# CUHK-SE-Group/MicroRank

Hardware: AMD Instinct MI355X
Metric: PageRank GTEPS + RCA windows ranked/sec at 1/2/4/8 MI355X; % HBM roofline (higher is better)
Workload: dtype f64

## Files before the change

microrank_amd/csrc/mr_graph_build.hip:

```cpp
#include <algorithm>
#include <cstring>
#include <vector>

#include "mr_detect_dev.h"
#include "mr_prim.h"
#include "mr_sort.h"

namespace {
constexpr int BT = 256;
constexpr int LDS_HIST = 8192;
constexpr int ESET = 1024;
constexpr uint64_t EMPTY = ~0ull;

__device__ __forceinline__ uint64_t hmix(uint64_t z) {
    z ^= z >> 33;
    z *= 0xff51afd7ed558ccdull;
    z ^= z >> 33;
    z *= 0xc4ceb9fe1a85ec53ull;
    return z ^ (z >> 33);
}

__global__ void k_count_codes(const int64_t* span, int64_t S, int32_t* cnt) {
    int64_t i = (int64_t)blockIdx.x * blockDim.x + threadIdx.x;
    if (i < S) atomicAdd(&cnt[span[i]], 1);
// ... 1920 lines not shown
    for (int k = 0; k < n; ++k) as.w[k].st = dst + woff[(size_t)k];
    if (fuse) {
        hipLaunchKernelGGL(k_ix_detect_scan2_b, dim3(bs), dim3(DB), 0, st, as, epoch);
    } else {
        if (dets) {
            int32_t bd = 0;
            IxBatch<IxWinSel> ad = as;
            for (int k = 0; k < n; ++k) {
                ad.b0[k] = bd;
                bd += (int32_t)cdiv((int64_t)sps[k]->n_traces, DB);
            }
            for (int k = n; k <= IXW; ++k) ad.b0[k] = bd;
            if (bd) hipLaunchKernelGGL(k_ix_detect_b, dim3(bd), dim3(DB), 0, st, ad);
        }
        hipLaunchKernelGGL(k_ix_sel_scan2_b, dim3(bs), dim3(SEL_T), 0, st, as, epoch);
    }
    if (bt) hipLaunchKernelGGL(k_ix_stats2_b, dim3(bt), dim3(IX_BT), lds, st, at);
    if (bc) hipLaunchKernelGGL(k_ix_cross2_b, dim3(bc), dim3(256), 0, st, ac);
    hipLaunchKernelGGL(k_nodes_small2_b, dim3(2 * n), dim3(NS_T), 0, st, an);
    if (br) hipLaunchKernelGGL(k_ix_traces2_b, dim3(br), dim3(256), 0, st, ar);
    MR_TRY_HIP(ctx, hipGetLastError());
    return MR_OK;
}

constexpr int LB_T = 512;
constexpr int64_t LB_LDS_WORDS = 30720;
constexpr int32_t LB_A3MAX = 4096;
bool mr_lo_fits(const mr_spans* sp) {
    return sp->indexed && sp->ekey.p && sp->n_podops <= NS_PMAX && sp->n_edge_keys <= NS_EMAX &&
           2 * (3 * (int64_t)sp->n_podops + sp->n_edge_keys) + 2 * (int64_t)sp->n_svcops <= LB_LDS_WORDS &&
           sp->n_svcops <= LB_A3MAX && sp->n_traces <= (1 << 24);
}
struct IxWinLoB {
    const int32_t *lo_tr, *lo_len, *lo_kid, *lo_first, *bstart;
    const int64_t *lo_off, *lsv_off, *le_off;
    const uint16_t *lo16, *lo_cnt;
    const uint32_t *lsv, *le;
    const long long *lo_ts, *lo_te, *lo_mx;
    const double* a3;
    const uint8_t* a3v;
    int64_t t0, t1;
    uint8_t* state;
    int8_t* side;
    unsigned long long* counts;
    int32_t NT, NP, nek, nsvc;
    uint32_t* kcnt[2];
    int64_t* tot[2];
    uint32_t* rows;
};
__host__ __device__ __forceinline__ size_t lo_region0(size_t gbytes) {
    return 2 * gbytes > (size_t)2048 * 8 ? 2 * gbytes : (size_t)2048 * 8;
}
constexpr int LB_R = 4;
__device__ __forceinline__ int32_t lo_trace_of(uint32_t e, uint32_t n, const uint32_t* st, int32_t nt) {
    if (n > 0) return (int32_t)(e / n);
    int32_t lo = 0;
#pragma unroll
    for (int32_t step = LO_BT_MAX / 2; step >= 1; step >>= 1) {
        const int32_t mid = lo + step;
        lo = mid < nt && st[mid] <= e ? mid : lo;
    }
    return lo;
}
__global__ void __launch_bounds__(LB_T, 6) k_lo_build_b(IxBatch<IxWinLoB> a) {
    extern __shared__ __attribute__((aligned(16))) unsigned char lraw[];
    __shared__ uint32_t pst[LO_BT_MAX + 1], est[LO_BT_MAX + 1];
    __shared__ int8_t ss[LO_BT_MAX];
    __shared__ unsigned long long bc[5][LB_T / WAVE];
    const int k = ixb_pick(a.b0, a.n);
    const IxWinLoB& w = a.w[k];
    const int32_t blk = (int32_t)blockIdx.x - a.b0[k];
    const int tid = threadIdx.x, lane = tid & (WAVE - 1), wv = tid / WAVE;
    const int32_t NP = w.NP, nek = w.nek;
    const size_t gbytes = ((size_t)NP * 12 + (size_t)nek * 4 + 15) / 16 * 16;
    const size_t reg0 = lo_region0(gbytes);
    double* la3 = (double*)(lraw + reg0);
    double* prod = (double*)lraw;
    const uint32_t cap = (uint32_t)(reg0 / 8 / LB_T * LB_T);
    for (int32_t c = tid; c < w.nsvc; c += LB_T) la3[c] = w.a3v[c] ? w.a3[c] : 0.0;
    const int32_t T0 = w.bstart[blk], nt = w.bstart[blk + 1] - T0;
    const int64_t P0 = w.lo_off[T0], Q0 = w.le_off[T0], V0 = w.lsv_off[T0];
    const uint32_t np = (uint32_t)(w.lo_off[T0 + nt] - P0), nq = (uint32_t)(w.le_off[T0 + nt] - Q0);
    const uint32_t nv = (uint32_t)(w.lsv_off[T0 + nt] - V0);
    if (tid == 0) {
        pst[nt] = np;
        est[nt] = nq;
    }
    constexpr int NS = LO_BT_MAX / LB_T;
    uint32_t va[NS], vb[NS];
    bool act[NS];
    double expect[NS];
    long long mx[NS];
    unsigned long long rows = 0;
#pragma unroll
    for (int q = 0; q < NS; ++q) {
        const int32_t t = q * LB_T + tid;
        const bool valid = t < nt;
        const int64_t i = (int64_t)T0 + (valid ? t : nt - 1);
        const int32_t len = w.lo_len[i];
        const long long ts = w.lo_ts[i], te = w.lo_te[i];
        mx[q] = w.lo_mx[i];
        va[q] = (uint32_t)(w.lsv_off[i] - V0);
        vb[q] = (uint32_t)(w.lsv_off[i + 1] - V0);
        const bool in = valid && len > 0 && ts >= w.t0 && te <= w.t1;
        rows += in ? (unsigned long long)len : 0ull;
        act[q] = in && mx[q] > 0;
        expect[q] = 0.0;
    }
    __syncthreads();
    for (uint32_t r0 = 0; r0 < nv; r0 += cap) {
        const uint32_t rn = min(cap, nv - r0);
        constexpr int LU = 8;
        for (uint32_t x0 = 0; x0 < rn; x0 += LU * LB_T) {
            uint32_t v[LU];
#pragma unroll
            for (int u = 0; u < LU; ++u) {
                const uint32_t x = x0 + (uint32_t)(u * LB_T + tid);
                v[u] = w.lsv[V0 + (int64_t)(r0 + min(x, rn - 1))];
            }
#pragma unroll
            for (int u = 0; u < LU; ++u) {
                const uint32_t x = x0 + (uint32_t)(u * LB_T + tid);
                if (x < rn) prod[x] = (double)(v[u] >> 16) * la3[v[u] & 0xffffu];
            }
        }
        __syncthreads();
#pragma unroll
        for (int q = 0; q < NS; ++q)
            if (act[q]) {
                const uint32_t lo = max(va[q], r0), hi = min(vb[q], r0 + rn);
                for (uint32_t j = lo; j < hi; j += 8) {
                    double p8[8];
#pragma unroll
                    for (int u = 0; u < 8; ++u) p8[u] = prod[min(j + u, hi - 1) - r0];
#pragma unroll
                    for (int u = 0; u < 8; ++u)
                        if (j + u < hi) expect[q] += p8[u];
                }
            }
        __syncthreads();
    }
    for (size_t x = (size_t)tid * 4; x < reg0; x += (size_t)LB_T * 4) *(uint32_t*)(lraw + x) = 0u;
    unsigned long long nab = 0, nno = 0, nz0 = 0, nz1 = 0;
#pragma unroll
    for (int q = 0; q < NS; ++q) {
        const int32_t t = q * LB_T + tid;
        const bool valid = t < nt;
        const int64_t i = (int64_t)T0 + (valid ? t : nt - 1);
        const int32_t kid0 = w.lo_kid[i], tr = w.lo_tr[i];
        const int64_t pa = w.lo_off[i], pb = w.lo_off[i + 1], ea = w.le_off[i];
        const int stt = act[q] ? ((double)mx[q] / 1000.0 > expect[q] ? 2 : 1) : 0;
        const int s_ = valid ? (stt == 2 ? 0 : stt == 1 ? 1 : -1) : -1;
        if (valid) {
            w.state[tr] = (uint8_t)stt;
            w.side[i] = (int8_t)s_;
            ss[t] = (int8_t)s_;
            pst[t] = (uint32_t)(pa - P0);
            est[t] = (uint32_t)(ea - Q0);
        }
        nab += stt == 2;
        nno += stt == 1;
        if (s_ == 0) nz0 += (unsigned long long)(pb - pa);
        else if (s_ == 1) nz1 += (unsigned long long)(pb - pa);
        const int kid = valid ? kid0 : -1;
        const int kp = __shfl_up(kid, 1, WAVE);
        const bool hd = kid >= 0 && (lane == 0 || kp != kid);
        const unsigned long long H = __ballot(hd), B0 = __ballot(s_ == 0), B1 = __ballot(s_ == 1);
        if (hd) {
            const unsigned long long above = lane == WAVE - 1 ? 0ull : H & (~0ull << (lane + 1));
            const unsigned long long run = (above ? (above & (0ull - above)) - 1ull : ~0ull) & (~0ull << lane);
            const uint32_t c0 = (uint32_t)__popcll(B0 & run), c1 = (uint32_t)__popcll(B1 & run);
            if (c0) atomicAdd(&w.kcnt[0][kid], c0);
            if (c1) atomicAdd(&w.kcnt[1][kid], c1);
        }
    }
    __syncthreads();
    constexpr int LB_LANE = 8;
    const bool lanewise = nt > 0 && pst[nt] - pst[nt - 1] <= (uint32_t)LB_LANE;
    if (lanewise) {
#pragma unroll
        for (int q = 0; q < NS; ++q) {
            const int32_t t = q * LB_T + tid;
            const int sd = t < nt ? (int)ss[t] : -1;
            if (sd < 0) continue;
            unsigned char* G = lraw + (size_t)sd * gbytes;
            const uint32_t a0 = pst[t], n = pst[t + 1] - a0, rot = n ? (uint32_t)t % n : 0u;
            uint32_t pc[LB_LANE];
            int32_t fr[LB_LANE];
#pragma unroll
            for (int u = 0; u < LB_LANE; ++u) {
                const uint32_t j = (uint32_t)u + rot;
                const int64_t e = P0 + (int64_t)a0 + (u < (int)n ? (j >= n ? j - n : j) : 0u);
                pc[u] = (uint32_t)w.lo16[e] | ((uint32_t)w.lo_cnt[e] << 16);
                fr[u] = w.lo_first[e];
            }
#pragma unroll
            for (int u = 0; u < LB_LANE; ++u)
                if (u < (int)n) {
                    const uint32_t c = pc[u] & 0xffffu;
                    atomicAdd((unsigned long long*)G + c, (unsigned long long)(pc[u] >> 16) | (1ull << 32));
                    atomicMax((int32_t*)(G + (size_t)NP * 8) + c, 0x7fffffff - fr[u]);
                }
            const uint32_t b0e = est[t], m = est[t + 1] - b0e, rte = m ? (uint32_t)t % m : 0u;
            uint32_t* Ge = (uint32_t*)(G + (size_t)NP * 12);
            for (uint32_t u0 = 0; u0 < m; u0 += LB_LANE) {
                uint32_t ev[LB_LANE];
#pragma unroll
                for (int u = 0; u < LB_LANE; ++u) {
                    const uint32_t j = u0 + (uint32_t)u, jr = j + rte;
                    ev[u] = w.le[Q0 + (int64_t)b0e + (j < m ? (jr >= m ? jr - m : jr) : 0u)];
                }
#pragma unroll
                for (int u = 0; u < LB_LANE; ++u)
                    if (u0 + (uint32_t)u < m) atomicAdd(Ge + (ev[u] & 0xffffu), ev[u] >> 16);
            }
        }
    }
    const uint32_t n0 = nt ? pst[1 < nt ? 1 : nt] - pst[0] : 0u;
    const uint32_t npo = n0 > 0 && np == (uint32_t)nt * n0 ? n0 : 0u;
    constexpr int NW = LB_T / WAVE;
    const uint32_t nmax = lanewise ? 0u : max(np, nq);
    for (uint32_t b0 = (uint32_t)wv * (LB_R * WAVE); b0 < nmax; b0 += NW * LB_R * WAVE) {
        uint32_t pc[LB_R], ev[LB_R];
        int32_t fr[LB_R];
#pragma unroll
        for (int r = 0; r < LB_R; ++r) {
            const uint32_t o = b0 + (uint32_t)(r * WAVE + lane);
            if (b0 < np) {
                const int64_t e = P0 + (int64_t)min(o, np - 1u);
                pc[r] = (uint32_t)w.lo16[e] | ((uint32_t)w.lo_cnt[e] << 16);
                fr[r] = w.lo_first[e];
            }
            if (b0 < nq) ev[r] = w.le[Q0 + (int64_t)min(o, nq - 1u)];
        }
#pragma unroll
        for (int r = 0; r < LB_R; ++r) {
            const uint32_t o = b0 + (uint32_t)(r * WAVE + lane);
            if (o < np) {
                const int sd = ss[lo_trace_of(o, npo, pst, nt)];
                if (sd >= 0) {
                    unsigned char* G = lraw + (size_t)sd * gbytes;
                    const uint32_t c = pc[r] & 0xffffu;
                    atomicAdd((unsigned long long*)G + c, (unsigned long long)(pc[r] >> 16) | (1ull << 32));
                    atomicMax((int32_t*)(G + (size_t)NP * 8) + c, 0x7fffffff - fr[r]);
                }
            }
            if (o < nq) {
                const int sd = ss[lo_trace_of(o, 0u, est, nt)];
                if (sd >= 0)
                    atomicAdd((uint32_t*)(lraw + (size_t)sd * gbytes + (size_t)NP * 12) + (ev[r] & 0xffffu), ev[r] >> 16);
            }
        }
    }
    __syncthreads();
    {
        unsigned long long v[5] = {nab, nno, rows, nz0, nz1};
#pragma unroll
        for (int m = 32; m >= 1; m >>= 1)
#pragma unroll
            for (int q = 0; q < 5; ++q) v[q] += __shfl_xor(v[q], m, WAVE);
        if (lane == 0)
#pragma unroll
            for (int q = 0; q < 5; ++q) bc[q][wv] = v[q];
    }
    __syncthreads();
    if (tid < 5) {
        unsigned long long v = 0;
        for (int q = 0; q < NW; ++q) v += bc[tid][q];
        if (v) {
            if (tid < 3) atomicAdd(&w.counts[(size_t)(blk % CSH) * 3 + tid], v);
            else atomicAdd((unsigned long long*)&w.tot[tid - 3][1], v);
        }
    }
    const size_t rw = 3 * (size_t)NP + (size_t)nek;
    uint32_t* R = w.rows + (size_t)blk * 2 * rw;
    for (int g = 0; g < 2; ++g) {
        const unsigned char* G = lraw + (size_t)g * gbytes;
        uint32_t* Rg = R + (size_t)g * rw;
// ... 170 lines not shown
            ap.w[k].tot[j] = out + 5;
            L.kcnt[j] = B.kcnt;
            L.tot[j] = out + 5;
            IxLoRed& R = ar.w[k];
            R.ocnt[j] = ocnt;
            R.ofinv[j] = ofinv;
            R.ocov[j] = ocov;
            R.gc[j] = gc;
        }
        const int32_t nt = sp->lo_nblk;
        const int64_t rw = 3 * (int64_t)NP + nek;
        roff[(size_t)k] = rwords;
        rwords += (int64_t)nt * 2 * rw;
        ar.w[k].nblk = nt;
        ar.w[k].NP = NP;
        ar.w[k].nek = (int32_t)nek;
        ar.b0[k] = br;
        br += (int32_t)cdiv(2 * rw, 256);
        const int32_t npb = (int32_t)std::max<int64_t>(cdiv((int64_t)NT, LP_TILE), 1);
        woff[(size_t)k] = words;
        words += 2 * (int64_t)npb;
        ap.b0[k] = bp;
        bp += npb;
        ap.w[k].NT = NT;
        soff[(size_t)k] = sbytes;
        sbytes += ((int64_t)NT + 15) / 16 * 16;
        ab.b0[k] = bb;
        bb += nt;
        const DetIn& d = dets[k];
        L.bstart = sp->lo_bstart.p;
        L.lo_tr = sp->lo_tr.p;
        L.lo_len = sp->lo_len.p;
        L.lo_kid = sp->lo_kid.p;
        L.lo_first = sp->lo_first.p;
        L.lo_off = sp->lo_off.p;
        L.lsv_off = sp->lsv_off.p;
        L.le_off = sp->le_off.p;
        L.lo16 = sp->lo16.p;
        L.lo_cnt = sp->lo_cnt.p;
        L.lsv = sp->lsv.p;
        L.le = sp->le.p;
        L.lo_ts = sp->lo_ts.p;
        L.lo_te = sp->lo_te.p;
        L.lo_mx = sp->lo_mx.p;
        L.a3 = d.a3;
        L.a3v = d.a3v;
        L.t0 = d.t0;
        L.t1 = d.t1;
        L.state = d.state;
        L.counts = d.counts;
        L.NT = NT;
        L.NP = NP;
        L.nek = (int32_t)nek;
        L.nsvc = sp->n_svcops;
        lds = std::max(lds, lo_region0(((size_t)NP * 12 + (size_t)nek * 4 + 15) / 16 * 16) + (size_t)sp->n_svcops * 8);
        ac.b0[k] = bc;
        bc += (int32_t)cdiv(sp->n_xj, 256);
        ac.w[k] = IxWinCross{d.state, sp->xj_tc.p, sp->xj_tp.p, sp->xj_eid.p, sp->n_xj, xs};
        an.b0[k] = 2 * k;
        an.w[k] = IxWinNodes{sp->ekey.p, nek, NP, 0, na};
    }
    for (int k = n; k <= IXW; ++k) {
        ab.b0[k] = bb;
        ar.b0[k] = br;
        ap.b0[k] = bp;
        ac.b0[k] = bc;
        an.b0[k] = 2 * n;
    }
    unsigned long long* dst = nullptr;
    uint64_t epoch = 0;
    MR_TRY(mr_dl_status(ctx, words, &dst, &epoch));
    DBuf<uint32_t> rows;
    DBuf<int8_t> side;
    MR_TRY(rows.alloc(ctx, (size_t)std::max<int64_t>(rwords, 1)));
    MR_TRY(side.alloc(ctx, (size_t)std::max<int64_t>(sbytes, 16)));
    for (int k = 0; k < n; ++k) {
        ab.w[k].rows = rows.p + roff[(size_t)k];
        ar.w[k].rows = rows.p + roff[(size_t)k];
        ab.w[k].side = side.p + soff[(size_t)k];
        ap.w[k].side = side.p + soff[(size_t)k];
        ap.w[k].st = dst + woff[(size_t)k];
    }
    hipLaunchKernelGGL(k_lo_build_b, dim3(bb), dim3(LB_T), lds, st, ab);
    hipLaunchKernelGGL(k_lo_pos_b, dim3(bp), dim3(LP_T), 0, st, ap, epoch);
    hipLaunchKernelGGL(k_lo_reduce_b, dim3(br), dim3(256), 0, st, ar);
    if (bc) hipLaunchKernelGGL(k_ix_cross2_b, dim3(bc), dim3(256), 0, st, ac);
    hipLaunchKernelGGL(k_nodes_small2_b, dim3(2 * n), dim3(NS_T), 0, st, an);
    MR_TRY_HIP(ctx, hipGetLastError());
// ... 112 lines not shown
```

microrank_amd/csrc/mr_internal.h:

```cpp
#pragma once
#include <hip/hip_runtime.h>

#include <cstdarg>
#include <cstdint>
#include <cstdio>
#include <map>
#include <string>
#include <unordered_map>
#include <utility>
#include <memory>
#include <mutex>
#include <vector>

#include "../../include/microrank_hip.h"

constexpr int WAVE = 64;

struct mr_ctx {
    int device = 0;
    hipStream_t stream = nullptr;
    uint32_t flags = 0;
    std::string err;
    void* comm = nullptr;
    int rank = 0, nranks = 1;
// ... 236 lines not shown
    mr_ctx* ctx = nullptr;
    int64_t S = 0;
    int32_t n_traces = 0, n_podops = 0, n_svcops = 0;
    DBuf<int32_t> trace, podop, svcop;
    DBuf<int64_t> span, parent, duration, tstart, tend;
    bool has_times = false;
    DBuf<int32_t> grow;
    int row_bits = 0;
    int64_t n_span_codes = 0;
    DBuf<int64_t> id_off;
    DBuf<int32_t> id_rows;
    bool indexed = false;
    bool uniform_times = false;
    DBuf<int32_t> tlen;
    DBuf<long long> tmaxd, tts, tte;
    int64_t n_po = 0, n_sv = 0, n_ed = 0, n_xj = 0;
    int64_t n_edge_keys = 0;
    DBuf<uint64_t> ekey;
    DBuf<int32_t> ed_eid, xj_eid;
    DBuf<int64_t> po_off;
    DBuf<int32_t> po_op, po_cnt, po_first, po_tr;
    DBuf<int64_t> sv_off;
    DBuf<int32_t> sv_op, sv_cnt;
    DBuf<int64_t> ed_off;
    DBuf<uint64_t> ed_key;
    DBuf<int32_t> ed_cnt, ed_tr;
    DBuf<int32_t> eb_tr, eb_cnt, eb_eid;
    DBuf<int32_t> xj_tc, xj_tp;
    DBuf<uint64_t> xj_key;
    bool lo_ok = false;
    int32_t lo_nk = 0;
    DBuf<int32_t> lo_tr, lo_len, lo_kid;
    DBuf<int64_t> lo_off;
    DBuf<uint16_t> lo16, lo_cnt;
    DBuf<int32_t> lo_first;
    DBuf<long long> lo_ts, lo_te, lo_mx;
    DBuf<int32_t> lo_bstart;
    int32_t lo_nblk = 0;
    DBuf<int64_t> lsv_off, le_off;
    DBuf<uint32_t> lsv, le;
    DBuf<int32_t> dict_rows[3];
    bool raw = false;
    DBuf<int64_t> raw_off[6];
    DBuf<uint8_t> raw_bytes[6], raw_valid;
    DBuf<int64_t> src;
    int64_t src_next = 0;
};

int mr_spans_index(mr_ctx* ctx, mr_spans* s);

void mr_handle_add(mr_ctx* ctx, void* h, void (*del)(void*));
bool mr_handle_take(void* h);

enum { MR_DT_F64 = 0, MR_DT_I32 = 1, MR_DT_U64 = 2, MR_DT_I64 = 3 };
int mr_coll_allreduce(mr_ctx* ctx, void* dbuf, int64_t n, int dtype, int op );
int mr_coll_allgather(mr_ctx* ctx, const void* dsend, void* drecv, int64_t n, int dtype);
inline bool mr_coll_ready(const mr_ctx* ctx) { return ctx->comm || ctx->host_coll; }
int mr_peer_allreduce_u64(mr_ctx* ctx, unsigned long long* dbuf, int64_t n);
int mr_peer_allreduce_f64(mr_ctx* ctx, double* dbuf, int64_t n);
int mr_peer_check(mr_ctx* ctx, const char* what);
struct MrPeerX {
    unsigned long long* const* peers;
    unsigned long long* region;
    int32_t R, rank, nbf, spin;
    int32_t mute;
    int64_t slots, W, bflags, err;
    uint64_t seq;
    unsigned long long timeout;
// ... 46 lines not shown
int mr_pagerank_batch_async(mr_ctx* ctx, mr_graph* const* gs, const int* anomaly, int ng, double d, double alpha,
                            int iters, int precision, int32_t* hflag, PrAsync** out, bool defer = false);
int mr_pagerank_async_commit(mr_ctx* ctx, PrAsync* a);
int mr_pagerank_async_finish(mr_ctx* ctx, PrAsync* a, bool* rerun);
void mr_pagerank_async_free(PrAsync* a);
int mr_ix_launch2_batch(mr_ctx* ctx, int n, const mr_spans* const* sps, uint8_t* const* d_states, mr_graph* const* g0s,
                        mr_graph* const* g1s, IxBuild* const* b0s, IxBuild* const* b1s, int64_t* const* d_outs,
                        const DetIn* dets, bool fuse);
constexpr int MR_DETECT_SHARDS = 64;
int mr_detect_indexed_launch(mr_ctx* ctx, const mr_spans* s, int64_t t0, int64_t t1, const double* d_a3,
                             const uint8_t* d_a3v, uint8_t* d_state, unsigned long long* counts);
void mr_detect_sum(const unsigned long long* sh, int32_t* n_abn, int32_t* n_nor, int64_t* n_in);
int mr_detect_sweep_launch(mr_ctx* ctx, const mr_spans* s, int64_t t_begin, int64_t grain, int64_t window, int32_t M,
                           const double* d_a3, const uint8_t* d_a3v, uint8_t* d_state, unsigned long long* diff);
constexpr size_t MR_WS_SLOT = 12 * 256 + 16;
int mr_win_spectrum_launch(mr_ctx* ctx, int32_t Na, const int32_t* a_podop, const double* a_w, const int32_t* a_cov,
                           int32_t Nn, const int32_t* n_podop, const double* n_w, const int32_t* n_cov, int32_t NP,
                           int64_t A, int64_t Nl, int method, int32_t k, unsigned char* d_slot);
void mr_win_spectrum_unpack(const unsigned char* slot, int32_t* out_codes, double* out_score, int32_t* n_out);
constexpr int MR_WS_BATCH = 8;
struct MrWsWin {
    const int32_t *a_podop, *a_cov, *n_podop, *n_cov;
    const double *a_w, *n_w;
    unsigned char* out;
    int64_t A, Nl;
    int32_t Na, Nn, NP;
};
bool mr_win_spectrum_fits(int32_t Na, int32_t Nn, int32_t NP, int32_t k);
int mr_win_spectrum_launch_n(mr_ctx* ctx, const MrWsWin* ws, int n, int method, int32_t k);
int mr_ix_finish(mr_ctx* ctx, const mr_spans* sp, mr_graph* g, IxBuild& b, const int64_t* h);
bool mr_lo_fits(const mr_spans* sp);
constexpr int32_t LO_BT_MAX = 1024;
constexpr int64_t LO_BE = 12288;
int64_t mr_lo_zero_words(const mr_spans* sp);
int mr_lo_launch_batch(mr_ctx* ctx, int n, const mr_spans* const* sps, mr_graph* const* g0s, mr_graph* const* g1s,
                       IxBuild* const* b0s, IxBuild* const* b1s, int64_t* const* d_outs, const DetIn* dets,
                       uint32_t* const* zw);
int mr_lo_prepare_batch(mr_ctx* ctx, mr_graph* const* gs, const mr_spans* const* sps, IxBuild* const* bs,
                        const int* anomaly, int n, double d, int precision, std::vector<unsigned char>& keep);
int mr_ix_finish_unprepared(mr_ctx* ctx, const mr_spans* sp, mr_graph* g, IxBuild& b, const int64_t* h);
int mr_pagerank_presetup(mr_ctx* ctx, mr_graph* g, int anomaly, double d, int precision, uint32_t flags);
int mr_pagerank_presetup_n(mr_ctx* ctx, mr_graph* const* gs, const int* anomaly, int n, double d, int precision,
                           std::vector<unsigned char>& keep);
```

microrank_amd/csrc/mr_span_index.hip:

```cpp
#include <algorithm>
#include <climits>
#include <cstring>

#include "mr_detect_dev.h"
#include "mr_prim.h"
#include "mr_sort.h"

namespace {
constexpr int XB = 256;

__global__ void k_ix_keys(const int32_t* trace, const int32_t* code, int64_t S, int nbc, uint64_t* key, uint32_t* val) {
    const int64_t i = (int64_t)blockIdx.x * blockDim.x + threadIdx.x;
    if (i >= S) return;
    key[i] = ((uint64_t)(uint32_t)trace[i] << nbc) | (uint32_t)code[i];
    val[i] = (uint32_t)i;
}
__global__ void k_ix_heads(const uint64_t* key, int64_t n, int32_t* head) {
    const int64_t i = (int64_t)blockIdx.x * blockDim.x + threadIdx.x;
    if (i < n) head[i] = (i == 0 || key[i] != key[i - 1]) ? 1 : 0;
}
__global__ void k_ix_runs(const uint64_t* key, const uint32_t* val, const int32_t* head, const int64_t* hpos, int64_t n,
                          int nbc, int32_t* r_code, int32_t* r_first, int32_t* r_tr, int64_t* r_start, int32_t* truns) {
    const int64_t i = (int64_t)blockIdx.x * blockDim.x + threadIdx.x;
    if (i >= n || !head[i]) return;
// ... 162 lines not shown
    if (t >= NT) return;
    const int64_t o = po_off[t], n = po_off[t + 1] - o;
    uint64_t acc = 0;
    for (int64_t e = 0; e < n; ++e) acc += lo_mix((uint64_t)po_op[o + e] ^ seed);
    hkey[t] = lo_mix(lo_mix(seed ^ (uint64_t)__float_as_uint(lo_w(tlen[t])) ^ ((uint64_t)n << 32)) + acc);
    tr[t] = (uint32_t)t;
}
__global__ void k_lo_keys(const uint32_t* tr_h, const int64_t* po_off, int32_t NT, int nbt, uint64_t* key) {
    const int32_t j = blockIdx.x * blockDim.x + threadIdx.x;
    if (j >= NT) return;
    const uint32_t t = tr_h[j];
    key[j] = ((uint64_t)(po_off[t + 1] - po_off[t]) << nbt) | (uint32_t)j;
}
__global__ void k_lo_unpack(const uint64_t* key, const uint32_t* tr_h, const uint64_t* hkey_h, int32_t NT, int nbt,
                            const int32_t* tlen, int32_t* lo_tr, int32_t* lo_n, int32_t* lo_len, int32_t* head) {
    const int32_t i = blockIdx.x * blockDim.x + threadIdx.x;
    if (i >= NT) return;
    const uint64_t m = (1ull << nbt) - 1ull, k = key[i];
    const uint32_t j = (uint32_t)(k & m);
    const int32_t t = (int32_t)tr_h[j];
    lo_tr[i] = t;
    lo_n[i] = (int32_t)(k >> nbt);
    lo_len[i] = tlen[t];
    bool h = i == 0;
    if (!h) {
        const uint64_t kp = key[i - 1];
        h = (kp >> nbt) != (k >> nbt) || hkey_h[(uint32_t)(kp & m)] != hkey_h[j];
    }
    head[i] = h ? 1 : 0;
}
__global__ void k_lo_copy(const int32_t* lo_tr, const int64_t* lo_off, int32_t NT, const int64_t* po_off,
                          const int32_t* po_op, const int32_t* po_cnt, const int32_t* po_first, const long long* tts,
                          const long long* tte, const long long* tmaxd, const int64_t* sv_off, const int64_t* ed_off,
                          uint16_t* lo16, uint16_t* lo_cnt, int32_t* lo_first, long long* lo_ts, long long* lo_te,
                          long long* lo_mx, int32_t* nsv, int32_t* ned, int32_t* bad) {
    const int32_t i = blockIdx.x * blockDim.x + threadIdx.x;
    if (i >= NT) return;
    const int32_t t = lo_tr[i];
    const int64_t a = po_off[t], n = po_off[t + 1] - a, o = lo_off[i];
    bool big = false;
    for (int64_t e = 0; e < n; ++e) {
        const int32_t c = po_cnt[a + e];
        big = big || c > 65535;
        lo16[o + e] = (uint16_t)po_op[a + e];
        lo_cnt[o + e] = (uint16_t)c;
        lo_first[o + e] = po_first[a + e];
    }
    lo_ts[i] = tts[t];
    lo_te[i] = tte[t];
    lo_mx[i] = tmaxd[t];
    nsv[i] = (int32_t)(sv_off[t + 1] - sv_off[t]);
    ned[i] = (int32_t)(ed_off[t + 1] - ed_off[t]);
    if (big) atomicOr(bad, 1);
}
__global__ void k_lo_copy2(const int32_t* lo_tr, int32_t NT, const int64_t* sv_off, const int32_t* sv_op,
                           const int32_t* sv_cnt, const int64_t* ed_off, const int32_t* ed_eid, const int32_t* ed_cnt,
                           const int64_t* lsv_off, const int64_t* le_off, uint32_t* lsv, uint32_t* le, int32_t* bad) {
    const int32_t i = blockIdx.x * blockDim.x + threadIdx.x;
    if (i >= NT) return;
    const int32_t t = lo_tr[i];
    bool big = false;
    for (int64_t e = sv_off[t], o = lsv_off[i]; e < sv_off[t + 1]; ++e, ++o) {
        const int32_t op = sv_op[e], c = sv_cnt[e];
        big = big || op > 65535 || c > 65535;
        lsv[o] = (uint32_t)(uint16_t)op | ((uint32_t)(uint16_t)c << 16);
    }
    for (int64_t e = ed_off[t], o = le_off[i]; e < ed_off[t + 1]; ++e, ++o) {
        const int32_t id = ed_eid[e], c = ed_cnt[e];
        big = big || id > 65535 || c > 65535;
        le[o] = (uint32_t)(uint16_t)id | ((uint32_t)(uint16_t)c << 16);
    }
    if (big) atomicOr(bad, 1);
}
__global__ void k_lo_reps(const int32_t* head, const int64_t* hpos, int32_t NT, int32_t* rep) {
    const int32_t i = blockIdx.x * blockDim.x + threadIdx.x;
    if (i < NT && head[i]) rep[hpos[i]] = i;
}
__global__ void k_lo_classes(const int32_t* head, const int64_t* hpos, const int32_t* rep, int32_t NT,
                             const int64_t* lo_off, const uint16_t* lo16, const int32_t* lo_len, int32_t* lo_kid,
// ... 129 lines not shown
static int lo_index_try(mr_ctx* ctx, mr_spans* s) {
    hipStream_t st = ctx->stream;
    const int32_t NT = s->n_traces;
    s->lo_ok = false;
    if (getenv("MR_LO_TEST_FAIL")) {
        MR_TRY(s->lo_tr.alloc(ctx, (size_t)std::max(NT, 1)));
        return mr_fail(ctx, MR_ERR_HIP, "lo_index: forced failure (MR_LO_TEST_FAIL)");
    }
    if (!mr_lo_fits(s) || s->n_po >= ((int64_t)1 << 31) || s->n_sv >= ((int64_t)1 << 31) ||
        s->n_ed >= ((int64_t)1 << 31))
        return MR_OK;
    const int nbt = std::max(1, bits_for((uint64_t)std::max(NT - 1, 0)));
    const int nbn = bits_for((uint64_t)s->n_podops);
    DBuf<uint64_t> hkey, key;
    DBuf<uint32_t> tr_h;
    DBuf<int32_t> lo_n, nsv, ned, head, rep, bad;
    DBuf<int64_t> hpos, tmp;
    MR_TRY(hkey.alloc(ctx, (size_t)NT));
    MR_TRY(rep.alloc(ctx, (size_t)NT));
    MR_TRY(key.alloc(ctx, (size_t)NT));
    MR_TRY(tr_h.alloc(ctx, (size_t)NT));
    MR_TRY(lo_n.alloc(ctx, (size_t)NT));
    MR_TRY(nsv.alloc(ctx, (size_t)NT));
    MR_TRY(ned.alloc(ctx, (size_t)NT));
    MR_TRY(head.alloc(ctx, (size_t)NT));
    MR_TRY(hpos.alloc(ctx, (size_t)NT + 1));
    MR_TRY(tmp.alloc(ctx, (size_t)scan_tmp_elems(NT)));
    MR_TRY(bad.alloc(ctx, 1));
    MR_TRY(s->lo_tr.alloc(ctx, (size_t)NT));
    MR_TRY(s->lo_len.alloc(ctx, (size_t)NT));
    MR_TRY(s->lo_kid.alloc(ctx, (size_t)NT));
    MR_TRY(s->lo_off.alloc(ctx, (size_t)NT + 1));
    MR_TRY(s->lo16.alloc(ctx, (size_t)std::max<int64_t>(s->n_po, 1)));
    MR_TRY(s->lo_cnt.alloc(ctx, (size_t)std::max<int64_t>(s->n_po, 1)));
    MR_TRY(s->lo_first.alloc(ctx, (size_t)std::max<int64_t>(s->n_po, 1)));
    MR_TRY(s->lo_ts.alloc(ctx, (size_t)NT));
    MR_TRY(s->lo_te.alloc(ctx, (size_t)NT));
    MR_TRY(s->lo_mx.alloc(ctx, (size_t)NT));
    MR_TRY(s->lsv_off.alloc(ctx, (size_t)NT + 1));
    MR_TRY(s->le_off.alloc(ctx, (size_t)NT + 1));
    MR_TRY(s->lsv.alloc(ctx, (size_t)std::max<int64_t>(s->n_sv, 1)));
    MR_TRY(s->le.alloc(ctx, (size_t)std::max<int64_t>(s->n_ed, 1)));
    const bool collide = getenv("MR_KIND_TEST_COLLIDE") != nullptr;
    for (int attempt = 0; attempt < 4; ++attempt) {
        const uint64_t seed = 0x51ed270b27a3c0deull + 0x9E3779B97F4A7C15ull * (uint64_t)attempt;
        MR_TRY(bad.zero(ctx, 1));
        hipLaunchKernelGGL(k_lo_hash, dim3(cdiv(NT, XB)), dim3(XB), 0, st, s->po_off.p, s->po_op.p, s->tlen.p, NT, seed,
                           hkey.p, tr_h.p);
        if (collide && attempt == 0) MR_TRY_HIP(ctx, hipMemsetAsync(hkey.p, 0, (size_t)NT * 8, st));
        SortScratch ws;
        MR_TRY(mr_radix_sort(ctx, hkey.p, tr_h.p, NT, 64, ws));
        hipLaunchKernelGGL(k_lo_keys, dim3(cdiv(NT, XB)), dim3(XB), 0, st, tr_h.p, s->po_off.p, NT, nbt, key.p);
        MR_TRY(mr_radix_sort(ctx, key.p, nullptr, NT, nbt + nbn, ws));
        hipLaunchKernelGGL(k_lo_unpack, dim3(cdiv(NT, XB)), dim3(XB), 0, st, key.p, tr_h.p, hkey.p, NT, nbt, s->tlen.p,
                           s->lo_tr.p, lo_n.p, s->lo_len.p, head.p);
        MR_TRY(mr_exclusive_scan_i32(ctx, lo_n.p, s->lo_off.p, NT, tmp.p));
        hipLaunchKernelGGL(k_lo_copy, dim3(cdiv(NT, XB)), dim3(XB), 0, st, s->lo_tr.p, s->lo_off.p, NT, s->po_off.p,
                           s->po_op.p, s->po_cnt.p, s->po_first.p, s->tts.p, s->tte.p, s->tmaxd.p, s->sv_off.p,
                           s->ed_off.p, s->lo16.p, s->lo_cnt.p, s->lo_first.p, s->lo_ts.p, s->lo_te.p, s->lo_mx.p, nsv.p,
                           ned.p, bad.p);
        int32_t hb = 0;
        MR_TRY(bad.download(ctx, &hb, 1));
        MR_TRY_HIP(ctx, hipStreamSynchronize(st));
        if (hb) return MR_OK;
        MR_TRY(mr_exclusive_scan_i32(ctx, head.p, hpos.p, NT, tmp.p));
        hipLaunchKernelGGL(k_lo_reps, dim3(cdiv(NT, XB)), dim3(XB), 0, st, head.p, hpos.p, NT, rep.p);
        hipLaunchKernelGGL(k_lo_classes, dim3(cdiv(NT, XB)), dim3(XB), 0, st, head.p, hpos.p, rep.p, NT, s->lo_off.p,
                           s->lo16.p, s->lo_len.p, s->lo_kid.p, bad.p);
        MR_TRY_HIP(ctx, hipGetLastError());
        int64_t nk = 0;
        MR_TRY_HIP(ctx, hipMemcpyAsync(&nk, hpos.p + NT, sizeof nk, hipMemcpyDeviceToHost, st));
        MR_TRY(bad.download(ctx, &hb, 1));
        MR_TRY_HIP(ctx, hipStreamSynchronize(st));
        if (hb) continue;
        MR_TRY(mr_exclusive_scan_i32(ctx, nsv.p, s->lsv_off.p, NT, tmp.p));
        MR_TRY(mr_exclusive_scan_i32(ctx, ned.p, s->le_off.p, NT, tmp.p));
        hipLaunchKernelGGL(k_lo_copy2, dim3(cdiv(NT, XB)), dim3(XB), 0, st, s->lo_tr.p, NT, s->sv_off.p, s->sv_op.p,
                           s->sv_cnt.p, s->ed_off.p, s->ed_eid.p, s->ed_cnt.p, s->lsv_off.p, s->le_off.p, s->lsv.p,
                           s->le.p, bad.p);
        MR_TRY_HIP(ctx, hipGetLastError());
        MR_TRY(bad.download(ctx, &hb, 1));
        MR_TRY_HIP(ctx, hipStreamSynchronize(st));
        if (hb) return MR_OK;
        {
            std::vector<int64_t> off((size_t)NT + 1);
            MR_TRY(s->lo_off.download(ctx, off.data(), (size_t)NT + 1));
            MR_TRY_HIP(ctx, hipStreamSynchronize(st));
            std::vector<int32_t> bs;
            bs.push_back(0);
            for (int32_t i = 0; i < NT; ++i) {
                const int32_t b0 = bs.back();
                if (i > b0 && (i - b0 >= LO_BT_MAX || off[(size_t)i + 1] - off[(size_t)b0] > LO_BE)) bs.push_back(i);
            }
            bs.push_back(NT);
            MR_TRY(s->lo_bstart.upload(ctx, bs.data(), bs.size()));
            MR_TRY_HIP(ctx, hipStreamSynchronize(st));
            s->lo_nblk = (int32_t)bs.size() - 1;
        }
        s->lo_nk = (int32_t)nk;
        s->lo_ok = true;
        return MR_OK;
    }
    return MR_OK;
}
static void lo_release(mr_spans* s) {
    s->lo_ok = false;
    s->lo_nk = 0;
    s->lo_nblk = 0;
    s->lo_tr.reset();
    s->lo_len.reset();
    s->lo_kid.reset();
    s->lo_off.reset();
    s->lo16.reset();
    s->lo_cnt.reset();
    s->lo_first.reset();
    s->lo_ts.reset();
    s->lo_te.reset();
    s->lo_mx.reset();
    s->lo_bstart.reset();
    s->lsv_off.reset();
    s->le_off.reset();
    s->lsv.reset();
    s->le.reset();
}
static int lo_index(mr_ctx* ctx, mr_spans* s) {
    const int rc = lo_index_try(ctx, s);
    if (rc != MR_OK) {
        (void)hipStreamSynchronize(ctx->stream);
        (void)hipGetLastError();
        ctx->err.clear();
    }
    if (rc != MR_OK || !s->lo_ok) lo_release(s);
    return MR_OK;
}

int mr_spans_index(mr_ctx* ctx, mr_spans* s) {
    hipStream_t st = ctx->stream;
    const int64_t S = s->S;
    const int32_t NT = s->n_traces, NP = s->n_podops;
    s->indexed = false;
    const int nbt = bits_for((uint64_t)std::max(NT - 1, 0));
    const int nbp = std::max(1, bits_for((uint64_t)std::max(NP - 1, 0)));
    const int nbs = std::max(1, bits_for((uint64_t)std::max(s->n_svcops - 1, 0)));
    if (S == 0 || NT == 0 || nbt + 2 * nbp > 64 || nbt + nbs > 64 || nbp > 32) return MR_OK;
    MR_TRY(s->tlen.zero(ctx, NT));
    MR_TRY(s->tmaxd.alloc(ctx, NT));
    MR_TRY(s->tts.alloc(ctx, NT));
    MR_TRY(s->tte.alloc(ctx, NT));
// ... 178 lines not shown
```

Baseline: 1068.

## Pack pod-op records into u64 and hoist per-trace loads in lo build kernel

```diff
diff --git a/microrank_amd/csrc/mr_graph_build.hip b/microrank_amd/csrc/mr_graph_build.hip
--- a/microrank_amd/csrc/mr_graph_build.hip
+++ b/microrank_amd/csrc/mr_graph_build.hip
@@ -1976,9 +1976,9 @@
            sp->n_svcops <= LB_A3MAX && sp->n_traces <= (1 << 24);
 }
 struct IxWinLoB {
-    const int32_t *lo_tr, *lo_len, *lo_kid, *lo_first, *bstart;
+    const int32_t *lo_tr, *lo_len, *lo_kid, *bstart;
     const int64_t *lo_off, *lsv_off, *le_off;
-    const uint16_t *lo16, *lo_cnt;
+    const uint64_t* lo_rec;
     const uint32_t *lsv, *le;
     const long long *lo_ts, *lo_te, *lo_mx;
     const double* a3;
@@ -1995,8 +1995,16 @@
 __host__ __device__ __forceinline__ size_t lo_region0(size_t gbytes) {
     return 2 * gbytes > (size_t)2048 * 8 ? 2 * gbytes : (size_t)2048 * 8;
 }
+__host__ __device__ __forceinline__ bool lo_a3_inside(size_t reg0, int32_t nsvc) {
+    return reg0 >= (size_t)nsvc * 8 + (size_t)2048 * 8;
+}
+__host__ __device__ __forceinline__ size_t lo_lds_bytes(size_t gbytes, int32_t nsvc) {
+    const size_t reg0 = lo_region0(gbytes);
+    return lo_a3_inside(reg0, nsvc) ? reg0 : reg0 + (size_t)nsvc * 8;
+}
 constexpr int LB_R = 4;
-__device__ __forceinline__ int32_t lo_trace_of(uint32_t e, uint32_t n, const uint32_t* st, int32_t nt) {
+template <class U>
+__device__ __forceinline__ int32_t lo_trace_of(uint32_t e, uint32_t n, const U* st, int32_t nt) {
     if (n > 0) return (int32_t)(e / n);
     int32_t lo = 0;
 #pragma unroll
@@ -2006,9 +2014,16 @@
     }
     return lo;
 }
+__device__ __forceinline__ void lo_rec_add(unsigned char* G, int32_t NP, uint64_t rc) {
+    const uint32_t c = (uint32_t)rc & 0xffffu;
+    atomicAdd((unsigned long long*)G + c, (unsigned long long)(((uint32_t)rc >> 16) & 0xffffu) | (1ull << 32));
+    atomicMax((int32_t*)(G + (size_t)NP * 8) + c, 0x7fffffff - (int32_t)(uint32_t)(rc >> 32));
+}
 __global__ void __launch_bounds__(LB_T, 6) k_lo_build_b(IxBatch<IxWinLoB> a) {
     extern __shared__ __attribute__((aligned(16))) unsigned char lraw[];
-    __shared__ uint32_t pst[LO_BT_MAX + 1], est[LO_BT_MAX + 1];
+    static_assert(LO_BE + NS_PMAX <= 65535, "pst holds a range's pod-op entry offsets as u16");
+    __shared__ uint16_t pst[LO_BT_MAX + 1];
+    __shared__ uint32_t est[LO_BT_MAX + 1];
     __shared__ int8_t ss[LO_BT_MAX];
     __shared__ unsigned long long bc[5][LB_T / WAVE];
     const int k = ixb_pick(a.b0, a.n);
@@ -2018,34 +2033,60 @@
     const int32_t NP = w.NP, nek = w.nek;
     const size_t gbytes = ((size_t)NP * 12 + (size_t)nek * 4 + 15) / 16 * 16;
     const size_t reg0 = lo_region0(gbytes);
-    double* la3 = (double*)(lraw + reg0);
+    const size_t a3b = lo_a3_inside(reg0, w.nsvc) ? reg0 - (size_t)w.nsvc * 8 : reg0;
+    double* la3 = (double*)(lraw + a3b);
     double* prod = (double*)lraw;
-    const uint32_t cap = (uint32_t)(reg0 / 8 / LB_T * LB_T);
-    for (int32_t c = tid; c < w.nsvc; c += LB_T) la3[c] = w.a3v[c] ? w.a3[c] : 0.0;
+    const uint32_t cap = (uint32_t)(a3b / 8 / LB_T * LB_T);
     const int32_t T0 = w.bstart[blk], nt = w.bstart[blk + 1] - T0;
     const int64_t P0 = w.lo_off[T0], Q0 = w.le_off[T0], V0 = w.lsv_off[T0];
     const uint32_t np = (uint32_t)(w.lo_off[T0 + nt] - P0), nq = (uint32_t)(w.le_off[T0 + nt] - Q0);
     const uint32_t nv = (uint32_t)(w.lsv_off[T0 + nt] - V0);
+    constexpr int LB_LANE = 8;
+    const bool lanewise = nt > 0 && P0 + (int64_t)np - w.lo_off[T0 + (nt > 0 ? nt - 1 : 0)] <= (int64_t)LB_LANE;
     if (tid == 0) {
-        pst[nt] = np;
+        pst[nt] = (uint16_t)np;
         est[nt] = nq;
     }
     constexpr int NS = LO_BT_MAX / LB_T;
-    uint32_t va[NS], vb[NS];
+    uint32_t va[NS], vb[NS], pn[NS];
+    int32_t kid0[NS], trc[NS];
     bool act[NS];
     double expect[NS];
     long long mx[NS];
     unsigned long long rows = 0;
+    int32_t len_[NS];
+    long long ts_[NS], te_[NS];
+    int64_t sva[NS], svb[NS], pa_[NS], pb_[NS], ea_[NS];
+#pragma unroll
+    for (int q = 0; q < NS; ++q) {
+        const int32_t t = q * LB_T + tid;
+        const int64_t i = (int64_t)T0 + (t < nt ? t : nt - 1);
+        len_[q] = w.lo_len[i];
+        ts_[q] = w.lo_ts[i];
+        te_[q] = w.lo_te[i];
+        mx[q] = w.lo_mx[i];
+        sva[q] = w.lsv_off[i];
+        svb[q] = w.lsv_off[i + 1];
+        kid0[q] = w.lo_kid[i];
+        trc[q] = w.lo_tr[i];
+        pa_[q] = w.lo_off[i];
+        pb_[q] = w.lo_off[i + 1];
+        ea_[q] = w.le_off[i];
+    }
+    for (int32_t c = tid; c < w.nsvc; c += LB_T) la3[c] = w.a3v[c] ? w.a3[c] : 0.0;
 #pragma unroll
     for (int q = 0; q < NS; ++q) {
         const int32_t t = q * LB_T + tid;
         const bool valid = t < nt;
-        const int64_t i = (int64_t)T0 + (valid ? t : nt - 1);
-        const int32_t len = w.lo_len[i];
-        const long long ts = w.lo_ts[i], te = w.lo_te[i];
-        mx[q] = w.lo_mx[i];
-        va[q] = (uint32_t)(w.lsv_off[i] - V0);
-        vb[q] = (uint32_t)(w.lsv_off[i + 1] - V0);
+        const int32_t len = len_[q];
+        const long long ts = ts_[q], te = te_[q];
+        va[q] = (uint32_t)(sva[q] - V0);
+        vb[q] = (uint32_t)(svb[q] - V0);
+        pn[q] = (uint32_t)(pb_[q] - pa_[q]);
+        if (valid) {
+            pst[t] = (uint16_t)(pa_[q] - P0);
+            est[t] = (uint32_t)(ea_[q] - Q0);
+        }
         const bool in = valid && len > 0 && ts >= w.t0 && te <= w.t1;
         rows += in ? (unsigned long long)len : 0ull;
         act[q] = in && mx[q] > 0;
@@ -2090,23 +2131,18 @@
     for (int q = 0; q < NS; ++q) {
         const int32_t t = q * LB_T + tid;
         const bool valid = t < nt;
-        const int64_t i = (int64_t)T0 + (valid ? t : nt - 1);
-        const int32_t kid0 = w.lo_kid[i], tr = w.lo_tr[i];
-        const int64_t pa = w.lo_off[i], pb = w.lo_off[i + 1], ea = w.le_off[i];
         const int stt = act[q] ? ((double)mx[q] / 1000.0 > expect[q] ? 2 : 1) : 0;
         const int s_ = valid ? (stt == 2 ? 0 : stt == 1 ? 1 : -1) : -1;
         if (valid) {
-            w.state[tr] = (uint8_t)stt;
-            w.side[i] = (int8_t)s_;
+            w.state[trc[q]] = (uint8_t)stt;
+            w.side[(int64_t)T0 + t] = (int8_t)s_;
             ss[t] = (int8_t)s_;
-            pst[t] = (uint32_t)(pa - P0);
-            est[t] = (uint32_t)(ea - Q0);
         }
         nab += stt == 2;
         nno += stt == 1;
-        if (s_ == 0) nz0 += (unsigned long long)(pb - pa);
-        else if (s_ == 1) nz1 += (unsigned long long)(pb - pa);
-        const int kid = valid ? kid0 : -1;
+        if (s_ == 0) nz0 += (unsigned long long)pn[q];
+        else if (s_ == 1) nz1 += (unsigned long long)pn[q];
+        const int kid = valid ? kid0[q] : -1;
         const int kp = __shfl_up(kid, 1, WAVE);
         const bool hd = kid >= 0 && (lane == 0 || kp != kid);
         const unsigned long long H = __ballot(hd), B0 = __ballot(s_ == 0), B1 = __ballot(s_ == 1);
@@ -2119,44 +2155,43 @@
         }
     }
     __syncthreads();
-    constexpr int LB_LANE = 8;
-    const bool lanewise = nt > 0 && pst[nt] - pst[nt - 1] <= (uint32_t)LB_LANE;
     if (lanewise) {
+        uint64_t lr[NS][LB_LANE];
+        int sdq[NS];
 #pragma unroll
         for (int q = 0; q < NS; ++q) {
             const int32_t t = q * LB_T + tid;
-            const int sd = t < nt ? (int)ss[t] : -1;
+            sdq[q] = t < nt ? (int)ss[t] : -1;
+            if (sdq[q] < 0) continue;
+            const uint32_t a0 = pst[t], n = pst[t + 1] - a0, rot = n ? (uint32_t)t % n : 0u;
+#pragma unroll
+            for (int u = 0; u < LB_LANE; ++u) {
+                const uint32_t j = (uint32_t)u + rot;
+                lr[q][u] = w.lo_rec[P0 + (int64_t)a0 + (u < (int)n ? (j >= n ? j - n : j) : 0u)];
+            }
+        }
+#pragma unroll
+        for (int q = 0; q < NS; ++q) {
+            const int32_t t = q * LB_T + tid;
+            const int sd = sdq[q];
             if (sd < 0) continue;
             unsigned char* G = lraw + (size_t)sd * gbytes;
-            const uint32_t a0 = pst[t], n = pst[t + 1] - a0, rot = n ? (uint32_t)t % n : 0u;
-            uint32_t pc[LB_LANE];
-            int32_t fr[LB_LANE];
-#pragma unroll
-            for (int u = 0; u < LB_LANE; ++u) {
-                const uint32_t j = (uint32_t)u + rot;
-                const int64_t e = P0 + (int64_t)a0 + (u < (int)n ? (j >= n ? j - n : j) : 0u);
-                pc[u] = (uint32_t)w.lo16[e] | ((uint32_t)w.lo_cnt[e] << 16);
-                fr[u] = w.lo_first[e];
-            }
+            const uint32_t n = pst[t + 1] - pst[t];
 #pragma unroll
             for (int u = 0; u < LB_LANE; ++u)
-                if (u < (int)n) {
-                    const uint32_t c = pc[u] & 0xffffu;
-                    atomicAdd((unsigned long long*)G + c, (unsigned long long)(pc[u] >> 16) | (1ull << 32));
-                    atomicMax((int32_t*)(G + (size_t)NP * 8) + c, 0x7fffffff - fr[u]);
-                }
+                if (u < (int)n) lo_rec_add(G, NP, lr[q][u]);
             const uint32_t b0e = est[t], m = est[t + 1] - b0e, rte = m ? (uint32_t)t % m : 0u;
             uint32_t* Ge = (uint32_t*)(G + (size_t)NP * 12);
             for (uint32_t u0 = 0; u0 < m; u0 += LB_LANE) {
-                uint32_t ev[LB_LANE];
+                uint32_t le8[LB_LANE];
 #pragma unroll
                 for (int u = 0; u < LB_LANE; ++u) {
                     const uint32_t j = u0 + (uint32_t)u, jr = j + rte;
-                    ev[u] = w.le[Q0 + (int64_t)b0e + (j < m ? (jr >= m ? jr - m : jr) : 0u)];
+                    le8[u] = w.le[Q0 + (int64_t)b0e + (j < m ? (jr >= m ? jr - m : jr) : 0u)];
                 }
 #pragma unroll
                 for (int u = 0; u < LB_LANE; ++u)
-                    if (u0 + (uint32_t)u < m) atomicAdd(Ge + (ev[u] & 0xffffu), ev[u] >> 16);
+                    if (u0 + (uint32_t)u < m) atomicAdd(Ge + (le8[u] & 0xffffu), le8[u] >> 16);
             }
         }
     }
@@ -2165,16 +2200,12 @@
     constexpr int NW = LB_T / WAVE;
     const uint32_t nmax = lanewise ? 0u : max(np, nq);
     for (uint32_t b0 = (uint32_t)wv * (LB_R * WAVE); b0 < nmax; b0 += NW * LB_R * WAVE) {
-        uint32_t pc[LB_R], ev[LB_R];
-        int32_t fr[LB_R];
+        uint64_t rc[LB_R];
+        uint32_t ev[LB_R];
 #pragma unroll
         for (int r = 0; r < LB_R; ++r) {
             const uint32_t o = b0 + (uint32_t)(r * WAVE + lane);
-            if (b0 < np) {
-                const int64_t e = P0 + (int64_t)min(o, np - 1u);
-                pc[r] = (uint32_t)w.lo16[e] | ((uint32_t)w.lo_cnt[e] << 16);
-                fr[r] = w.lo_first[e];
-            }
+            if (b0 < np) rc[r] = w.lo_rec[P0 + (int64_t)min(o, np - 1u)];
             if (b0 < nq) ev[r] = w.le[Q0 + (int64_t)min(o, nq - 1u)];
         }
 #pragma unroll
@@ -2182,12 +2213,7 @@
             const uint32_t o = b0 + (uint32_t)(r * WAVE + lane);
             if (o < np) {
                 const int sd = ss[lo_trace_of(o, npo, pst, nt)];
-                if (sd >= 0) {
-                    unsigned char* G = lraw + (size_t)sd * gbytes;
-                    const uint32_t c = pc[r] & 0xffffu;
-                    atomicAdd((unsigned long long*)G + c, (unsigned long long)(pc[r] >> 16) | (1ull << 32));
-                    atomicMax((int32_t*)(G + (size_t)NP * 8) + c, 0x7fffffff - fr[r]);
-                }
+                if (sd >= 0) lo_rec_add(lraw + (size_t)sd * gbytes, NP, rc[r]);
             }
             if (o < nq) {
                 const int sd = ss[lo_trace_of(o, 0u, est, nt)];
@@ -2424,12 +2450,10 @@
         L.lo_tr = sp->lo_tr.p;
         L.lo_len = sp->lo_len.p;
         L.lo_kid = sp->lo_kid.p;
-        L.lo_first = sp->lo_first.p;
         L.lo_off = sp->lo_off.p;
         L.lsv_off = sp->lsv_off.p;
         L.le_off = sp->le_off.p;
-        L.lo16 = sp->lo16.p;
-        L.lo_cnt = sp->lo_cnt.p;
+        L.lo_rec = sp->lo_rec.p;
         L.lsv = sp->lsv.p;
         L.le = sp->le.p;
         L.lo_ts = sp->lo_ts.p;
@@ -2445,7 +2469,7 @@
         L.NP = NP;
         L.nek = (int32_t)nek;
         L.nsvc = sp->n_svcops;
-        lds = std::max(lds, lo_region0(((size_t)NP * 12 + (size_t)nek * 4 + 15) / 16 * 16) + (size_t)sp->n_svcops * 8);
+        lds = std::max(lds, lo_lds_bytes(((size_t)NP * 12 + (size_t)nek * 4 + 15) / 16 * 16, sp->n_svcops));
         ac.b0[k] = bc;
         bc += (int32_t)cdiv(sp->n_xj, 256);
         ac.w[k] = IxWinCross{d.state, sp->xj_tc.p, sp->xj_tp.p, sp->xj_eid.p, sp->n_xj, xs};
diff --git a/microrank_amd/csrc/mr_internal.h b/microrank_amd/csrc/mr_internal.h
--- a/microrank_amd/csrc/mr_internal.h
+++ b/microrank_amd/csrc/mr_internal.h
@@ -292,8 +292,8 @@
     int32_t lo_nk = 0;
     DBuf<int32_t> lo_tr, lo_len, lo_kid;
     DBuf<int64_t> lo_off;
-    DBuf<uint16_t> lo16, lo_cnt;
-    DBuf<int32_t> lo_first;
+    DBuf<uint16_t> lo16;
+    DBuf<uint64_t> lo_rec;
     DBuf<long long> lo_ts, lo_te, lo_mx;
     DBuf<int32_t> lo_bstart;
     int32_t lo_nblk = 0;
@@ -406,6 +406,9 @@
 bool mr_lo_fits(const mr_spans* sp);
 constexpr int32_t LO_BT_MAX = 1024;
 constexpr int64_t LO_BE = 12288;
+__host__ __device__ __forceinline__ uint64_t lo_rec_pack(uint16_t code, uint16_t cnt, int32_t first) {
+    return (uint64_t)code | (uint64_t)cnt << 16 | (uint64_t)(uint32_t)first << 32;
+}
 int64_t mr_lo_zero_words(const mr_spans* sp);
 int mr_lo_launch_batch(mr_ctx* ctx, int n, const mr_spans* const* sps, mr_graph* const* g0s, mr_graph* const* g1s,
                        IxBuild* const* b0s, IxBuild* const* b1s, int64_t* const* d_outs, const DetIn* dets,
diff --git a/microrank_amd/csrc/mr_span_index.hip b/microrank_amd/csrc/mr_span_index.hip
--- a/microrank_amd/csrc/mr_span_index.hip
+++ b/microrank_amd/csrc/mr_span_index.hip
@@ -218,7 +218,7 @@
 __global__ void k_lo_copy(const int32_t* lo_tr, const int64_t* lo_off, int32_t NT, const int64_t* po_off,
                           const int32_t* po_op, const int32_t* po_cnt, const int32_t* po_first, const long long* tts,
                           const long long* tte, const long long* tmaxd, const int64_t* sv_off, const int64_t* ed_off,
-                          uint16_t* lo16, uint16_t* lo_cnt, int32_t* lo_first, long long* lo_ts, long long* lo_te,
+                          uint16_t* lo16, uint64_t* lo_rec, long long* lo_ts, long long* lo_te,
                           long long* lo_mx, int32_t* nsv, int32_t* ned, int32_t* bad) {
     const int32_t i = blockIdx.x * blockDim.x + threadIdx.x;
     if (i >= NT) return;
@@ -228,9 +228,9 @@
     for (int64_t e = 0; e < n; ++e) {
         const int32_t c = po_cnt[a + e];
         big = big || c > 65535;
-        lo16[o + e] = (uint16_t)po_op[a + e];
-        lo_cnt[o + e] = (uint16_t)c;
-        lo_first[o + e] = po_first[a + e];
+        const int32_t op = po_op[a + e];
+        lo16[o + e] = (uint16_t)op;
+        lo_rec[o + e] = lo_rec_pack((uint16_t)op, (uint16_t)c, po_first[a + e]);
     }
     lo_ts[i] = tts[t];
     lo_te[i] = tte[t];
@@ -426,8 +426,7 @@
     MR_TRY(s->lo_kid.alloc(ctx, (size_t)NT));
     MR_TRY(s->lo_off.alloc(ctx, (size_t)NT + 1));
     MR_TRY(s->lo16.alloc(ctx, (size_t)std::max<int64_t>(s->n_po, 1)));
-    MR_TRY(s->lo_cnt.alloc(ctx, (size_t)std::max<int64_t>(s->n_po, 1)));
-    MR_TRY(s->lo_first.alloc(ctx, (size_t)std::max<int64_t>(s->n_po, 1)));
+    MR_TRY(s->lo_rec.alloc(ctx, (size_t)std::max<int64_t>(s->n_po, 1)));
     MR_TRY(s->lo_ts.alloc(ctx, (size_t)NT));
     MR_TRY(s->lo_te.alloc(ctx, (size_t)NT));
     MR_TRY(s->lo_mx.alloc(ctx, (size_t)NT));
@@ -451,7 +450,7 @@
         MR_TRY(mr_exclusive_scan_i32(ctx, lo_n.p, s->lo_off.p, NT, tmp.p));
         hipLaunchKernelGGL(k_lo_copy, dim3(cdiv(NT, XB)), dim3(XB), 0, st, s->lo_tr.p, s->lo_off.p, NT, s->po_off.p,
                            s->po_op.p, s->po_cnt.p, s->po_first.p, s->tts.p, s->tte.p, s->tmaxd.p, s->sv_off.p,
-                           s->ed_off.p, s->lo16.p, s->lo_cnt.p, s->lo_first.p, s->lo_ts.p, s->lo_te.p, s->lo_mx.p, nsv.p,
+                           s->ed_off.p, s->lo16.p, s->lo_rec.p, s->lo_ts.p, s->lo_te.p, s->lo_mx.p, nsv.p,
                            ned.p, bad.p);
         int32_t hb = 0;
         MR_TRY(bad.download(ctx, &hb, 1));
@@ -506,8 +505,7 @@
     s->lo_kid.reset();
     s->lo_off.reset();
     s->lo16.reset();
-    s->lo_cnt.reset();
-    s->lo_first.reset();
+    s->lo_rec.reset();
     s->lo_ts.reset();
     s->lo_te.reset();
     s->lo_mx.reset();
```

Result: faster. 1082 (median of 6 runs) (+1.4%).
